# XinkeAE/Active-ORB-SLAM2

Hardware: AMD Instinct MI355X
Metric: frames/sec (extract+match+localBA) TUM 640x480 (higher is better)
Workload: dtype u8 (extract, match) + f64 (PoseOptimization, LocalBA)

## Files before the change

active-orb-slam2_amd/csrc/lba.hip:

```cpp
#include <dlfcn.h>

#include <chrono>
#include <cstdio>
#include <cstdlib>
#include <memory>
#include <numeric>
#include <atomic>
#include <condition_variable>
#include <functional>
#include <mutex>
#include <thread>

#include "lba_math.h"
#include "ldlt_reg.h"
#include "wave_ops.h"

namespace aos2 {

struct Cam {
    double fx, fy, cx, cy, bf;
    float bf_f;
    double delta_mono, delta_stereo;
};

// ... 64 lines not shown
    LdltForm ldlt_form;
    int hs_ld;
    LmState *st;
    const int32_t *abort_word;
    float *out_Tcw, *out_xyz;
    double *out_chi2;
    uint8_t *out_outlier;
};

static_assert(sizeof(LbaWin) == 520 && offsetof(LbaWin, st) == 472, "LbaWin's layout is fixed");

struct SchurTask {
    int32_t w;
    int32_t code;
};

typedef float flt4_t __attribute__((ext_vector_type(4)));
typedef int int4_t __attribute__((ext_vector_type(4)));
__device__ __forceinline__ void erec_load(const LbaWin &W, int a, flt4_t &lo, int4_t &hi)
{
    const EdgeRec *r = W.erec + a;
    lo = *reinterpret_cast<const flt4_t *>(r);
    hi = *(reinterpret_cast<const int4_t *>(r) + 1);
}
__device__ __forceinline__ void erec_store(const LbaWin &W, int a, flt4_t lo, int4_t hi)
{
    EdgeRec *r = W.erec + a;
    *reinterpret_cast<flt4_t *>(r) = lo;
    *(reinterpret_cast<int4_t *>(r) + 1) = hi;
}

__device__ inline bool lm_poll(LmState *st, const int32_t *abort_word, int seen = -1)
{
    st->polls++;
    if (st->stop_poll > 0) return true;
    const int a = seen >= 0 ? seen : abort_word ? __hip_atomic_load(abort_word, __ATOMIC_RELAXED, __HIP_MEMORY_SCOPE_SYSTEM) : 0;
    if (a || (st->stop_at_poll > 0 && st->polls >= st->stop_at_poll)) {
        st->stop_poll = st->polls;
        return true;
    }
    return false;
}

__device__ inline void lm_first_done(LmState *st, const int32_t *abort_word, int seen = -1)
{
    st->phase = 1;
    st->xmark = 0;
    if (lm_poll(st, abort_word, seen)) {
        st->phase = 3;
        return;
    }
    st->xmark = 1;
    st->n_active = 0;
}

template <int N>
__device__ __forceinline__ void workgroup_sum2(double v0, double v1, double *out0, double *out1)
{
    __shared__ double sh[2][N];
    sh[0][threadIdx.x] = v0;
    sh[1][threadIdx.x] = v1;
    __syncthreads();
#pragma unroll
    for (int s = N / 2; s > 0; s >>= 1) {
        if ((int)threadIdx.x < s) {
            sh[0][threadIdx.x] = sh[0][threadIdx.x] + sh[0][threadIdx.x + s];
            sh[1][threadIdx.x] = sh[1][threadIdx.x] + sh[1][threadIdx.x + s];
        }
        __syncthreads();
    }
    if (threadIdx.x == 0) {
        out0[blockIdx.x] = sh[0][0];
        out1[blockIdx.x] = sh[1][0];
    }
}

__global__ __launch_bounds__(256) void k_prepare(const LbaWin *__restrict__ wins, int stop_at_poll)
{
    const LbaWin &W = wins[blockIdx.y];
    const int i = blockIdx.x * 256 + threadIdx.x;
    if (i < W.n_poses) pose_from_Tcw(W.in_Tcw + 16 * (size_t)i, W.pose + 7 * (size_t)i);
    if (i < W.n_points)
        for (int d = 0; d < 3; ++d) W.point[3 * (size_t)i + d] = (double)W.in_xyz[3 * (size_t)i + d];
    if (i < W.n_edges) {
        for (int d = 0; d < 3; ++d) W.err[3 * (size_t)i + d] = 0.0;
        W.e_robust[i] = 1;
        W.e_level1[i] = 0;
        const int k = W.pt_k[i];
        const flt4_t lo = {W.in_obs[3 * (size_t)k], W.in_obs[3 * (size_t)k + 1], W.in_obs[3 * (size_t)k + 2], W.in_w[k]};
        const int4_t hi = {W.e_pose[k], W.pl_pos[k], (int)((W.e_stereo[k] ? kEdgeStereo : 0) | kEdgeRobust), 0};
        erec_store(W, i, lo, hi);
    }
    if (blockIdx.x == 0 && W.hs_ld == W.npad) {
        const int n = 6 * W.np, npad = W.npad;
        for (int q = threadIdx.x; q < (npad - n) * npad; q += 256) {
            const int r = n + q / npad, c = q % npad;
            W.Hs[(size_t)r * npad + c] = r == c ? 1.0 : 0.0;
        }
        for (int q = threadIdx.x; q < n * (npad - n); q += 256) {
            const int r = q / (npad - n), c = n + q % (npad - n);
            W.Hs[(size_t)r * npad + c] = 0.0;
        }
    }
    if (blockIdx.x == 0) {
        LmState *st = W.st;
        static_assert(sizeof(LmState) % 8 == 0, "LmState is cleared as 64-bit words");
        for (int k = threadIdx.x; k < (int)(sizeof(LmState) / 8); k += 256) reinterpret_cast<long long *>(st)[k] = 0;
        __syncthreads();
        if (threadIdx.x == 0) {
            st->iters_max[0] = W.iters1;
            st->iters_max[1] = W.iters2;
            st->polls = 1;
            st->stop_at_poll = stop_at_poll;
            st->n_active = W.n_edges;
            st->phase = 0;
            st->it = 0;
            if (st->iters_max[0] <= 0 || lm_poll(st, W.abort_word)) {
                st->iters_done[0] = 0;
                lm_first_done(st, W.abort_word);
            } else
                st->initp = 1;
        }
    }
}

__device__ __forceinline__ void edge_error(const Cam &cam, const double p[3], const double *obs, int stereo, double er[3])
{
    if (!stereo) {
        const double u = p[0] / p[2], v = p[1] / p[2];
        er[0] = obs[0] - (u * cam.fx + cam.cx);
        er[1] = obs[1] - (v * cam.fy + cam.cy);
        er[2] = 0;
    } else {
        const float invz = (float)(1.0 / p[2]);
        const double r0 = p[0] * invz * cam.fx + cam.cx;
        const double r1 = p[1] * invz * cam.fy + cam.cy;
        const double r2 = r0 - (double)__fmul_rn(cam.bf_f, invz);
        er[0] = obs[0] - r0;
        er[1] = obs[1] - r1;
        er[2] = obs[2] - r2;
    }
}

__device__ __forceinline__ double load_dev(const double *p)
{
    return __longlong_as_double((long long)__hip_atomic_load(reinterpret_cast<const unsigned long long *>(p), __ATOMIC_RELAXED,
                                                             __HIP_MEMORY_SCOPE_AGENT));
}
__device__ __forceinline__ void store_dev(double *p, double v)
{
    __hip_atomic_store(reinterpret_cast<unsigned long long *>(p), (unsigned long long)__double_as_longlong(v), __ATOMIC_RELAXED,
                       __HIP_MEMORY_SCOPE_AGENT);
}
__device__ __forceinline__ void canonical_sums(const LbaWin &W, bool with_scale, double &chi_out, double &scale_out)
{
    __shared__ double s_red[2][128];
    const int tid = threadIdx.x;
    if (tid < 128) {
        double c = 0, s2 = 0;
        for (int i0 = tid; i0 < W.nl; i0 += 128 * 16) {
            double v[16], w[16];
#pragma unroll
            for (int u = 0; u < 16; ++u) {
                const int i = i0 + 128 * u;
                v[u] = i < W.nl ? load_dev(W.part + i) : 0.0;
                w[u] = with_scale && i < W.nl ? load_dev(W.part + W.nl + i) : 0.0;
            }
#pragma unroll
            for (int u = 0; u < 16; ++u) {
                c += v[u];
                s2 += w[u];
            }
        }
        if (with_scale)
            for (int i = tid; i < 6 * W.np; i += 128) s2 += W.tmp[i];
        s_red[0][tid] = c;
        s_red[1][tid] = s2;
    }
    __syncthreads();
    for (int h = 64; h > 0; h >>= 1) {
        if (tid < h) {
            s_red[0][tid] += s_red[0][tid + h];
            s_red[1][tid] += s_red[1][tid + h];
        }
        __syncthreads();
    }
    chi_out = s_red[0][0];
    scale_out = s_red[1][0];
}
template <int NT>
__device__ __forceinline__ void lm_decide(const LbaWin &W)
{
    __shared__ int s_restore;
    LmState *st = W.st;
    const int flag_seen = threadIdx.x == 0 && W.abort_word ? __hip_atomic_load(W.abort_word, __ATOMIC_RELAXED, __HIP_MEMORY_SCOPE_SYSTEM) : 0;
    double tempChi, scale;
    canonical_sums(W, true, tempChi, scale);
    if (threadIdx.x == 0) {
        const int pass = st->phase == 0 ? 0 : 1;
        const bool ok2 = W.np == 0 || W.scal[3] != 0.0;
        if (!ok2) {
            tempChi = 1.7976931348623157e308;
            st->solver_failed++;
        }
        double rho = st->currentChi - tempChi;
        scale += 1e-3;
        rho /= scale;
        if (!ok2) rho = -1.0;
        const bool accepted = rho > 0 && isfinite(tempChi);
        if (st->ntr < 48) {
            st->tr_rho[st->ntr] = rho; st->tr_temp[st->ntr] = tempChi; st->tr_cur[st->ntr] = st->currentChi;
            st->tr_lambda[st->ntr] = st->lambda;
            st->ntr++;
        }
        if (accepted) {
            const double t3 = 2 * rho - 1;
            double alpha = 1. - t3 * t3 * t3;
            alpha = alpha < 2. / 3. ? alpha : 2. / 3.;
            const double scaleFactor = 1. / 3. > alpha ? 1. / 3. : alpha;
            st->lambda *= scaleFactor;
            st->ni = 2;
            st->currentChi = tempChi;
            st->err_at = 1;
        } else {
            st->lambda *= st->ni;
            st->ni *= 2;
            st->err_at = 2;
        }
        s_restore = accepted ? 0 : 1;
        st->qmax++;
        st->trials[pass]++;
        int lin = 0;
        const bool again = rho < 0 && st->qmax < 10 && !lm_poll(st, W.abort_word, flag_seen);
        if (!again) {
            bool term = st->qmax == 10 || rho == 0;
            if (!term) {
                if ((st->iniChi - st->currentChi) * 1e3 < st->iniChi)
                    st->nBad++;
                else
                    st->nBad = 0;
                term = st->nBad >= 3;
            }
            st->it++;
            bool more = st->it < st->iters_max[pass];
            if (more) more = !lm_poll(st, W.abort_word, flag_seen);
            if (more) more = !term;
            if (more) {
                st->qmax = 0;
                st->iniChi = st->currentChi;
                lin = accepted ? 1 : 0;
            } else {
                st->run = 0;
                st->iters_done[pass] = st->it;
                st->final_chi2 = st->currentChi;
                st->final_lambda = st->lambda;
                if (pass == 0)
                    lm_first_done(st, W.abort_word, flag_seen);
                else
                    st->phase = 3;
            }
        }
        st->lin = lin;
    }
    __syncthreads();
    if (s_restore)
        for (int i = threadIdx.x; i < W.est_n; i += NT) {
            const double trial = load_dev(W.pose + i);
            W.pose[i] = load_dev(W.bk + i);
            W.bk[i] = trial;
        }
}

template <int NT>
__device__ __forceinline__ void points_tail(const LbaWin &W)
{
    __shared__ int s_last;
    asm volatile("s_waitcnt vmcnt(0)" ::: "memory");
    __builtin_amdgcn_fence(__ATOMIC_RELEASE, "workgroup");
    __syncthreads();
    if (threadIdx.x == 0)
        s_last = __hip_atomic_fetch_add(&W.st->blocks_done, 1, __ATOMIC_RELAXED, __HIP_MEMORY_SCOPE_AGENT) == W.n_part - 1;
    __syncthreads();
    if (!s_last) return;
    __builtin_amdgcn_fence(__ATOMIC_ACQUIRE, "workgroup");
    if (threadIdx.x == 0) W.st->blocks_done = 0;
    lm_decide<NT>(W);
}

__device__ __forceinline__ void jac_pose(const Cam &cam, const double p[3], int stereo, double Jb[18])
{
    const double fx = cam.fx, fy = cam.fy, bf = cam.bf;
    const double iz = 1.0 / p[2], a = p[0] * iz, b = p[1] * iz, ab = a * b;
    Jb[0] = ab * fx;
    Jb[1] = -(1 + a * a) * fx;
    Jb[2] = b * fx;
    Jb[3] = -(iz * fx);
    Jb[4] = 0;
    Jb[5] = a * iz * fx;
    Jb[6] = (1 + b * b) * fy;
    Jb[7] = -(ab * fy);
    Jb[8] = -(a * fy);
    Jb[9] = 0;
    Jb[10] = -(iz * fy);
    Jb[11] = b * iz * fy;
#pragma unroll
    for (int i = 12; i < 18; ++i) Jb[i] = 0;
    if (stereo) {
        const double bfz2 = bf * (iz * iz);
        Jb[12] = Jb[0] - bfz2 * p[1];
        Jb[13] = Jb[1] + bfz2 * p[0];
        Jb[14] = Jb[2];
        Jb[15] = Jb[3];
        Jb[16] = 0;
        Jb[17] = Jb[5] - bfz2;
    }
}

__device__ __forceinline__ void jac_point(const Cam &cam, const double R[9], const double p[3], int stereo, double Ja[9])
{
    const double iz = 1.0 / p[2], a = p[0] * iz, b = p[1] * iz;
    const double fxz = cam.fx * iz, fyz = cam.fy * iz, afxz = a * fxz, bfyz = b * fyz;
#pragma unroll
    for (int c = 0; c < 3; ++c) {
        Ja[c] = afxz * R[6 + c] - fxz * R[c];
        Ja[3 + c] = bfyz * R[6 + c] - fyz * R[3 + c];
        Ja[6 + c] = 0;
    }
    if (stereo) {
        const double bfz2 = cam.bf * (iz * iz);
#pragma unroll
        for (int c = 0; c < 3; ++c) Ja[6 + c] = Ja[c] - bfz2 * R[6 + c];
    }
}

typedef double dbl4_t __attribute__((ext_vector_type(4)));
__device__ __forceinline__ void lrec_store(const LbaWin &W, int pos, const double p[3], double wo, int stereo, const double omr[3])
// ... 266 lines not shown
{
    const SchurTask tk = tasks[blockIdx.x];
    const LbaWin &W = wins[tk.w];
    if (!(solve ? W.st->run : W.st->initp)) return;
    const int l = tk.code * blockDim.x + threadIdx.x;
    const bool has = l < W.nl;
    int hp = 0, a0 = 0, a1 = 0, e0 = 0, e1 = 0;
    if (has) {
        hp = W.hpoint[l];
        e0 = W.pt_off[l];
        e1 = W.pt_off[l + 1];
        if (solve) {
            a0 = W.pl_off[l];
            a1 = W.pl_off[l + 1];
        }
    }
    const bool lds = walk_lds_bytes(W.n_poses, W.np) <= kWalkLdsBytes;
    if (lds) {
        walk_stage(W, walk_sm, solve != 0);
        if (has) points_walk_body<true>(W, l, solve, hp, a0, a1, e0, e1);
    } else if (has)
        points_walk_body<false>(W, l, solve, hp, a0, a1, e0, e1);
    if (solve) points_tail<128>(W);
}

__device__ __forceinline__ void edge_weights_of(const Cam &cam, const double er[3], double w, int robust, int stereo, double omr[3], double &wo)
{
    omr[0] = -(w * er[0]);
    omr[1] = -(w * er[1]);
    omr[2] = stereo ? -(w * er[2]) : 0.0;
    wo = w;
    if (robust) {
        double rho[2];
        robustify(edge_chi2(er, w, stereo ? 3 : 2), stereo ? cam.delta_stereo : cam.delta_mono, rho);
        wo = rho[1] * w;
        omr[0] *= rho[1];
        omr[1] *= rho[1];
        if (stereo) omr[2] *= rho[1];
    }
}
__device__ __forceinline__ void edge_weights(const LbaWin &W, int k, const double p[3], int stereo, double omr[3], double &wo)
{
    const double ob[3] = {(double)W.in_obs[3 * (size_t)k], (double)W.in_obs[3 * (size_t)k + 1], (double)W.in_obs[3 * (size_t)k + 2]};
    double er[3];
    edge_error(W.cam, p, ob, stereo, er);
    edge_weights_of(W.cam, er, (double)W.in_w[k], W.e_robust[k], stereo, omr, wo);
}

__device__ __forceinline__ void lin_points_body(const LbaWin &W, int blk)
{
    __shared__ double s_c[kLmBlock][kLmSlots][12 + 1];
    const int tid = threadIdx.x, ll = tid / kLmSlots, j = tid % kLmSlots;
    const int l = blk * kLmBlock + ll;
    const bool has = l < W.nl, leader = j == 0;
    double Xv[3] = {0, 0, 0};
    if (has) {
        const double *X = W.point + 3 * (size_t)W.hpoint[l];
        for (int r = 0; r < 3; ++r) Xv[r] = X[r];
    }
    double H[9] = {0, 0, 0, 0, 0, 0, 0, 0, 0}, bl[3] = {0, 0, 0};
    const int a0 = has ? W.pt_off[l] : 0, a1 = has ? W.pt_off[l + 1] : 0;
    for (int rd = 0; __syncthreads_or(a0 + kLmSlots * rd < a1); ++rd) {
        const int a = a0 + kLmSlots * rd + j;
        double cH[9] = {0, 0, 0, 0, 0, 0, 0, 0, 0}, cb[3] = {0, 0, 0};
        const int k = a < a1 ? W.pt_k[a] : -1;
        if (k >= 0 && !W.e_level1[k]) {
            const double *T = W.pose + 7 * (size_t)W.e_pose[k];
            const int stereo = W.e_stereo[k];
            double p[3], R[9];
            se3_map(T, Xv, p);
            rot_from_quat(T, R);
            double Ja[9];
            jac_point(W.cam, R, p, stereo, Ja);
            double omr[3], wo;
            edge_weights(W, k, p, stereo, omr, wo);
#pragma unroll
            for (int r = 0; r < 3; ++r) {
                cb[r] = Ja[r] * omr[0] + Ja[3 + r] * omr[1] + Ja[6 + r] * omr[2];
#pragma unroll
                for (int c = 0; c < 3; ++c) cH[r * 3 + c] = Ja[r] * wo * Ja[c] + Ja[3 + r] * wo * Ja[3 + c] + Ja[6 + r] * wo * Ja[6 + c];
            }
            const int pp = W.pl_pos[k];
            if (pp >= 0) lrec_store(W, pp, p, wo, stereo, omr);
        }
#pragma unroll
        for (int i = 0; i < 9; ++i) s_c[ll][j][i] = cH[i];
#pragma unroll
        for (int i = 0; i < 3; ++i) s_c[ll][j][9 + i] = cb[i];
        __syncthreads();
        if (leader) {
            const int m = min(kLmSlots, a1 - (a0 + kLmSlots * rd));
            for (int jj = 0; jj < m; ++jj) {
#pragma unroll
                for (int i = 0; i < 9; ++i) H[i] += s_c[ll][jj][i];
#pragma unroll
                for (int i = 0; i < 3; ++i) bl[i] += s_c[ll][jj][9 + i];
            }
        }
    }
    if (has && leader) {
        for (int i = 0; i < 9; ++i) W.Hll[9 * (size_t)l + i] = H[i];
        for (int i = 0; i < 3; ++i) W.b[6 * (size_t)W.np + 3 * (size_t)l + i] = bl[i];
    }
}

template <bool kLds>
__device__ __forceinline__ void lin_points_walk(const LbaWin &W, int l)
{
    const double *s_pose = walk_sm;
    const int e0 = W.pt_off[l], e1 = W.pt_off[l + 1];
    const double *X = W.point + 3 * (size_t)W.hpoint[l];
    const double Xv[3] = {X[0], X[1], X[2]};
    double H[9] = {0, 0, 0, 0, 0, 0, 0, 0, 0}, bl[3] = {0, 0, 0};
    for (int a = e0; a < e1; a += kWalkChunkLin) {
        flt4_t lo[kWalkChunkLin];
        int4_t hi[kWalkChunkLin];
        double T[kWalkChunkLin][7];
#pragma unroll
        for (int u = 0; u < kWalkChunkLin; ++u) erec_load(W, min(a + u, e1 - 1), lo[u], hi[u]);
#pragma unroll
        for (int u = 0; u < kWalkChunkLin; ++u)
#pragma unroll
            for (int i = 0; i < 7; ++i) T[u][i] = kLds ? s_pose[7 * hi[u].x + i] : W.pose[7 * (size_t)hi[u].x + i];
#pragma unroll
        for (int u = 0; u < kWalkChunkLin; ++u) {
            if (a + u >= e1) break;
            const uint32_t fl = (uint32_t)hi[u].z;
            if (fl & kEdgeLevel1) continue;
            const int stereo = fl & kEdgeStereo;
            const double ob[3] = {(double)lo[u].x, (double)lo[u].y, (double)lo[u].z};
            double p[3], R[9];
            se3_map(T[u], Xv, p);
            rot_from_quat(T[u], R);
            double Ja[9];
            jac_point(W.cam, R, p, stereo, Ja);
            double omr[3], wo;
            double res[3];
            edge_error(W.cam, p, ob, stereo, res);
            edge_weights_of(W.cam, res, (double)lo[u].w, (fl & kEdgeRobust) != 0, stereo, omr, wo);
#pragma unroll
            for (int r = 0; r < 3; ++r) {
                bl[r] += Ja[r] * omr[0] + Ja[3 + r] * omr[1] + Ja[6 + r] * omr[2];
#pragma unroll
                for (int c = 0; c < 3; ++c) H[r * 3 + c] += Ja[r] * wo * Ja[c] + Ja[3 + r] * wo * Ja[3 + c] + Ja[6 + r] * wo * Ja[6 + c];
            }
            if (hi[u].y >= 0) lrec_store(W, hi[u].y, p, wo, stereo, omr);
        }
    }
    asm volatile("" : "+v"(l));
    for (int i = 0; i < 9; ++i) W.Hll[9 * (size_t)l + i] = H[i];
    for (int i = 0; i < 3; ++i) W.b[6 * (size_t)W.np + 3 * (size_t)l + i] = bl[i];
}

template <int K, int NT = 256>
__device__ __forceinline__ double workgroup_sum_k256(double (&acc)[K], double *red , int n_items)
{
    const int row = threadIdx.x >> 4, wave = threadIdx.x >> 6;
    const int rows_used = min(NT / 16, (n_items + 15) >> 4);
    if (wave * 64 < n_items) {
        row_sums_scatter_f64<K>(acc);
        row_scatter_store<K>(acc, red + row * (K + 1));
    }
    __syncthreads();
    double sum = 0;
    if ((int)threadIdx.x < K)
        for (int r = 0; r < rows_used; ++r) sum += red[r * (K + 1) + threadIdx.x];
    return sum;
}

__device__ __forceinline__ void lin_poses_body(const LbaWin &W, int ph, int init)
{
    __shared__ double red[16 * 43];
    if (ph >= W.np) return;
    double T[7];
    {
        const double *Tp = W.pose + 7 * (size_t)W.hpose[ph];
#pragma unroll
        for (int i = 0; i < 7; ++i) T[i] = Tp[i];
    }
    if (threadIdx.x == 0) {
        double R[9];
        rot_from_quat(T, R);
#pragma unroll
        for (int i = 0; i < 9; ++i) W.Rl[9 * (size_t)ph + i] = R[i];
    }
    if (!init) return;
    double acc[42];
#pragma unroll
    for (int i = 0; i < 42; ++i) acc[i] = 0;
    for (int a = W.ps_off[ph] + threadIdx.x; a < W.ps_off[ph + 1]; a += 256) {
        const int k = W.ps_k[a];
        if (W.e_level1[k]) continue;
        const int stereo = W.e_stereo[k];
        double p[3], Jb[18], omr[3], wo;
        se3_map(T, W.point + 3 * (size_t)W.e_point[k], p);
        jac_pose(W.cam, p, stereo, Jb);
        edge_weights(W, k, p, stereo, omr, wo);
#pragma unroll
        for (int r = 0; r < 6; ++r) {
            acc[36 + r] += Jb[r] * omr[0] + Jb[6 + r] * omr[1] + Jb[12 + r] * omr[2];
#pragma unroll
            for (int c = 0; c < 6; ++c) acc[r * 6 + c] += Jb[r] * wo * Jb[c] + Jb[6 + r] * wo * Jb[6 + c] + Jb[12 + r] * wo * Jb[12 + c];
        }
    }
    const double sum = workgroup_sum_k256<42>(acc, red, W.ps_off[ph + 1] - W.ps_off[ph]);
    if (threadIdx.x < 36)
        W.Hpp[36 * (size_t)ph + threadIdx.x] = sum;
    else if (threadIdx.x < 42)
        W.b[6 * (size_t)ph + (threadIdx.x - 36)] = sum;
}

template <bool kWalk>
__global__ __launch_bounds__(256) __attribute__((amdgpu_waves_per_eu(3, 3))) void k_lin(const LbaWin *__restrict__ wins, const SchurTask *__restrict__ tasks, int init)
{
    const SchurTask tk = tasks[blockIdx.x];
    const LbaWin &W = wins[tk.w];
    if (!(init ? W.st->initp : W.st->lin)) return;
    const int blk = tk.code & 0x0fffffff;
    const bool keyframe = (tk.code >> 28) != 0;
    if (keyframe)
        lin_poses_body(W, blk, init);
    else if (kWalk) {
        const int l = blk * 256 + threadIdx.x;
        const bool has = l < W.nl;
        if (walk_lds_bytes(W.n_poses, W.np) <= kWalkLdsBytes) {
            walk_stage(W, walk_sm, false);
            if (has) lin_points_walk<true>(W, l);
        } else if (has)
            lin_points_walk<false>(W, l);
    } else
        lin_points_body(W, blk);
}

__global__ __launch_bounds__(1024) void k_lm_init(const LbaWin *__restrict__ wins)
{
    __shared__ double sh[1024];
    const LbaWin &W = wins[blockIdx.x];
    LmState *st = W.st;
    if (!st->initp) return;
    const int n6 = 6 * W.np, n = n6 + 3 * W.nl;
    double acc = 0;
    for (int i = threadIdx.x; i < n; i += 1024) {
        double v;
        if (i < n6)
            v = W.Hpp[36 * (size_t)(i / 6) + (i % 6) * 7];
        else {
            const int j = i - n6;
            v = W.Hll[9 * (size_t)(j / 3) + (j % 3) * 4];
        }
        acc = fmax(acc, fabs(v));
    }
    sh[threadIdx.x] = acc;
    __syncthreads();
    for (int s = 512; s > 0; s >>= 1) {
        if ((int)threadIdx.x < s) sh[threadIdx.x] = fmax(sh[threadIdx.x], sh[threadIdx.x + s]);
        __syncthreads();
    }
    for (int i = threadIdx.x; i < W.est_n; i += 1024) W.bk[i] = W.pose[i];
    double chi, unused;
    canonical_sums(W, false, chi, unused);
    if (threadIdx.x == 0) {
        st->currentChi = st->iniChi = chi;
        st->lambda = 1e-5 * sh[0];
        st->ni = 2;
        st->nBad = 0;
        st->it = 0;
        st->qmax = 0;
        st->initp = 0;
        st->lin = 0;
        st->run = 1;
        st->err_at = 1;
    }
}

constexpr int kSchurThreads = 256;
constexpr int kSchurDiag = 0, kSchurBig = 1, kSchurPack = 2;
__device__ __forceinline__ double sf(double a, double b, double c) { return a * b + c; }
template <bool kDiag>
__device__ __forceinline__ void schur_item(const LbaWin &W, int j, double lambda, int n6, const double *__restrict__ Ra_g,
                                           const double *__restrict__ Rb_g, double (&acc)[42])
{
    const int ka = W.it_ka[j], kb = W.it_kb[j], l = W.it_l[j];
    const dbl4_t rb = lrec_load(W, kb);
    const dbl4_t ra = kDiag ? rb : lrec_load(W, ka);
    double D[9], Dinv[9];
#pragma unroll
    for (int i = 0; i < 9; ++i) D[i] = W.Hll[9 * (size_t)l + i];
    D[0] += lambda; D[4] += lambda; D[8] += lambda;
    mat3_inverse(D, Dinv);
    double Ra[9], G[9];
#pragma unroll
    for (int i = 0; i < 9; ++i) Ra[i] = Ra_g[i];
    {
        double G0[9];
#pragma unroll
        for (int r = 0; r < 3; ++r)
#pragma unroll
            for (int c = 0; c < 3; ++c) G0[r * 3 + c] = sf(Ra[r * 3 + 2], Dinv[6 + c], sf(Ra[r * 3 + 1], Dinv[3 + c], Ra[r * 3] * Dinv[c]));
        if (kDiag) {
            const double *bl = W.b + n6 + 3 * (size_t)l;
            const double b0 = bl[0], b1 = bl[1], b2 = bl[2];
            const EdgeLin La = lrec_form(W.cam, ra);
            const double t[3] = {G0[0] * b0 + G0[1] * b1 + G0[2] * b2, G0[3] * b0 + G0[4] * b1 + G0[5] * b2, G0[6] * b0 + G0[7] * b1 + G0[8] * b2};
            double h[3];
            lrec_C(La, t, h);
            acc[36] += La.b * h[2] - h[1];
            acc[37] += h[0] - La.a * h[2];
            acc[38] += La.a * h[1] - La.b * h[0];
            acc[39] += La.iz * h[0];
            acc[40] += La.iz * h[1];
            acc[41] += La.iz * h[2];
        }
        double Rb[9];
#pragma unroll
        for (int i = 0; i < 9; ++i) Rb[i] = kDiag ? Ra[i] : Rb_g[i];
#pragma unroll
        for (int r = 0; r < 3; ++r)
#pragma unroll
            for (int c = 0; c < 3; ++c) G[r * 3 + c] = sf(G0[r * 3 + 2], Rb[c * 3 + 2], sf(G0[r * 3 + 1], Rb[c * 3 + 1], G0[r * 3] * Rb[c * 3]));
    }
    const EdgeLin La = lrec_form(W.cam, ra), Lb = kDiag ? La : lrec_form(W.cam, rb);
    double Q[9];
    {
        double CG[9];
#pragma unroll
        for (int c = 0; c < 3; ++c) {
            CG[c] = sf(La.C02, G[6 + c], La.C00 * G[c]);
            CG[3 + c] = sf(La.C12, G[6 + c], La.C11 * G[3 + c]);
            CG[6 + c] = sf(La.C22, G[6 + c], sf(La.C12, G[3 + c], La.C02 * G[c]));
        }
#pragma unroll
        for (int r = 0; r < 3; ++r) {
            Q[r * 3] = sf(CG[r * 3 + 2], Lb.C02, CG[r * 3] * Lb.C00);
            Q[r * 3 + 1] = sf(CG[r * 3 + 2], Lb.C12, CG[r * 3 + 1] * Lb.C11);
            Q[r * 3 + 2] = sf(CG[r * 3 + 2], Lb.C22, sf(CG[r * 3 + 1], Lb.C12, CG[r * 3] * Lb.C02));
        }
    }
    if (kDiag) {
        const double w = fabs(ra.w), fx2 = W.cam.fx * W.cam.fx, fy2 = W.cam.fy * W.cam.fy;
        const bool st = ra.w < 0.0;
        const double fs = st ? W.cam.fx : 0.0, c = st ? W.cam.bf * La.iz - La.a * W.cam.fx : 0.0;
        const double P00 = (fx2 + fs * fs) * w, P02 = (fs * c - La.a * fx2) * w, P11 = fy2 * w, P12 = -(La.b * fy2) * w;
        const double P22 = (La.a * La.a * fx2 + La.b * La.b * fy2 + c * c) * w;
        Q[0] -= P00; Q[2] -= P02; Q[4] -= P11; Q[5] -= P12; Q[6] -= P02; Q[7] -= P12; Q[8] -= P22;
    }
#pragma unroll
    for (int c = 0; c < 6; ++c) {
        double u[3];
#pragma unroll
        for (int r = 0; r < 3; ++r) {
            const double q0 = Q[r * 3], q1 = Q[r * 3 + 1], q2 = Q[r * 3 + 2];
            u[r] = c == 0 ? q1 - Lb.b * q2 : c == 1 ? Lb.a * q2 - q0 : c == 2 ? Lb.b * q0 - Lb.a * q1 : -(Lb.iz * Q[r * 3 + (c - 3)]);
        }
        acc[c] += u[1] - La.b * u[2];
        if (!kDiag || c >= 1) acc[6 + c] += La.a * u[2] - u[0];
        if (!kDiag || c >= 2) acc[12 + c] += La.b * u[0] - La.a * u[1];
        if (!kDiag || c >= 3) acc[18 + c] += -(La.iz * u[0]);
        if (!kDiag || c >= 4) acc[24 + c] += -(La.iz * u[1]);
        if (!kDiag || c >= 5) acc[30 + c] += -(La.iz * u[2]);
    }
    if (kDiag) {
        const double o[3] = {W.lomr[3 * (size_t)kb], W.lomr[3 * (size_t)kb + 1], W.lomr[3 * (size_t)kb + 2]};
        double bp[6] = {0, 0, 0, 0, 0, 0};
        lrec_bp(W.cam, ra, o, bp);
        acc[6] += bp[0]; acc[12] += bp[1]; acc[13] += bp[2]; acc[18] += bp[3]; acc[19] += bp[4]; acc[20] += bp[5];
    }
}

__device__ __forceinline__ void schur_store(const LbaWin &W, int i1, int i2, int e, double sum, double lambda)
{
    const bool diag = i1 == i2;
    if (e < 36) {
        double v = -sum;
        const int r = e / 6, c = e - 6 * r;
        if (diag && r == c) v += lambda;
        W.Hs[(size_t)(6 * i1 + r) * W.hs_ld + 6 * i2 + c] = v;
        if (!diag) W.Hs[(size_t)(6 * i2 + c) * W.hs_ld + 6 * i1 + r] = v;
    }
}

__global__ __launch_bounds__(kSchurThreads) __attribute__((amdgpu_waves_per_eu(3, 3)))
void k_schur(const LbaWin *__restrict__ wins, const SchurTask *__restrict__ tasks)
{
    constexpr int NT = kSchurThreads;
// ... 945 lines not shown
    W.erec = (EdgeRec *)(base + l.erec); W.npad = l.npad; W.ldlt_form = l.ldlt_form;
    W.hs_ld = l.npad;
    W.st = (LmState *)(base + l.st);
    W.abort_word = abort_word;
    W.out_Tcw = (float *)(base + l.out_Tcw); W.out_xyz = (float *)(base + l.out_xyz);
    W.out_outlier = base + l.out_outlier;
    W.out_chi2 = want_chi2 ? (double *)(base + l.out_chi2) : nullptr;
}


struct GroupDims {
    bool any_glob = false, any_reg = false;
    int mx_E = 0, mx_pts = 0, mx_npad_glob = 0, mx_npad_reg = 0;
    int walk_lds = 0;
    void add(const aos2_lba_problem_t &p, const Pass &S, const WinLayout &l)
    {
        if (S.np > 0) {
            if (l.ldlt_form == kLdltReg) {
                any_reg = true;
                mx_npad_reg = std::max(mx_npad_reg, l.npad);
            } else {
                any_glob = true;
                mx_npad_glob = std::max(mx_npad_glob, l.npad);
            }
        }
        mx_E = std::max(mx_E, p.n_edges);
        mx_pts = std::max(mx_pts, std::max(p.n_points, p.n_poses));
        if (walk_lds_bytes(p.n_poses, S.np) <= kWalkLdsBytes) walk_lds = std::max(walk_lds, walk_lds_bytes(p.n_poses, S.np));
    }
};

struct TaskLists {
    std::vector<SchurTask> schur, pts, lin;
    size_t size() const { return schur.size() + pts.size() + lin.size(); }
};

static void build_tasks(const std::vector<Pass> &passes, const std::vector<int> &ids, bool by_position, const LmLayout &lay, TaskLists &T, bool one_queue = false)
{
    auto wmap = [&](int k) { return by_position ? k : ids[k]; };
    std::vector<SchurTask> &tasks = T.schur;
    const int nwg = (int)ids.size();
    std::vector<int> order(nwg);
    std::iota(order.begin(), order.end(), 0);
    auto weight = [&](int k) { return passes[ids[k]].units.size(); };
    std::stable_sort(order.begin(), order.end(), [&](int a, int b) { return weight(a) > weight(b); });
    const int NX = nwg >= 8 && !one_queue ? 8 : 1;
    std::vector<std::vector<int>> xw(NX);
    std::vector<size_t> load(NX, 0);
    for (int k : order) {
        const int x = (int)(std::min_element(load.begin(), load.end()) - load.begin());
        xw[x].push_back(k);
        load[x] += weight(k);
    }
    std::vector<std::vector<SchurTask>> qx(NX);
    for (int x = 0; x < NX; ++x)
        for (size_t k = 0; k < xw[x].size(); k += 2) {
            const int a = xw[x][k], b = k + 1 < xw[x].size() ? xw[x][k + 1] : -1;
            const std::vector<int32_t> &ua = passes[ids[a]].units;
            static const std::vector<int32_t> none;
            const std::vector<int32_t> &ub = b >= 0 ? passes[ids[b]].units : none;
            for (size_t u = 0; u < std::max(ua.size(), ub.size()); ++u) {
                if (u < ua.size()) qx[x].push_back(SchurTask{wmap(a), ua[u]});
                if (u < ub.size()) qx[x].push_back(SchurTask{wmap(b), ub[u]});
            }
        }
    size_t mxq = 0;
    for (auto &q_ : qx) mxq = std::max(mxq, q_.size());
    tasks.assign(mxq * NX, SchurTask{-1, 0});
    for (int x = 0; x < NX; ++x)
        for (size_t k = 0; k < qx[x].size(); ++k) tasks[k * NX + x] = qx[x][k];
    int mx_pb = 0, mx_lb = 0, mx_k = 0;
    std::vector<int> npb(nwg), nlb(nwg);
    for (int k = 0; k < nwg; ++k) {
        const Pass &S = passes[ids[k]];
        npb[k] = lay.points_blocks(S);
        nlb[k] = lay.lin_blocks(S);
        mx_pb = std::max(mx_pb, npb[k]); mx_lb = std::max(mx_lb, nlb[k]); mx_k = std::max(mx_k, S.np);
    }
    T.pts.clear();
    T.lin.clear();
    for (int b = 0; b < mx_pb; ++b)
        for (int k = 0; k < nwg; ++k)
            if (b < npb[k]) T.pts.push_back(SchurTask{wmap(k), b});
    for (int b = 0; b < mx_lb; ++b)
        for (int k = 0; k < nwg; ++k)
            if (b < nlb[k]) T.lin.push_back(SchurTask{wmap(k), b});
    for (int kf = 0; kf < mx_k; ++kf)
        for (int k = 0; k < nwg; ++k)
            if (kf < passes[ids[k]].np) T.lin.push_back(SchurTask{wmap(k), (1 << 28) | kf});
}

struct DevTasks {
    const SchurTask *schur, *pts, *lin;
};
static DevTasks put_tasks(const TaskLists &T, uint8_t *host, const uint8_t *dev, size_t &o)
{
    DevTasks d;
    const std::vector<SchurTask> *lists[3] = {&T.schur, &T.pts, &T.lin};
    const SchurTask **where[3] = {&d.schur, &d.pts, &d.lin};
    for (int k = 0; k < 3; ++k) {
        *where[k] = (const SchurTask *)(dev + o);
        if (!lists[k]->empty()) memcpy(host + o, lists[k]->data(), sizeof(SchurTask) * lists[k]->size());
        o += sizeof(SchurTask) * lists[k]->size();
    }
    return d;
}

struct StreamSet {
    hipStream_t q, q2;
    hipEvent_t fork, join;
};
static StreamSet group_streams(const aos2_lba *s, int g)
{
    return g == 0 ? StreamSet{s->stream, s->stream2, s->ev_fork, s->ev_join} : StreamSet{s->stream_b, s->stream2_b, s->ev_fork_b, s->ev_join_b};
}

struct Prog : StreamSet {
    const LbaWin *wins, *blk;
    int nw;
    const SchurTask *schur, *pts, *lin;
    size_t n_schur, n_pts, n_lin;
    GroupDims D;
};
static Prog make_prog(const LbaWin *wins, const LbaWin *blk, int nw, const TaskLists &T, const DevTasks &d, const GroupDims &D, const StreamSet &Q)
{
    return Prog{Q, wins, blk, nw, d.schur, d.pts, d.lin, T.schur.size(), T.pts.size(), T.lin.size(), D};
}

struct LaunchCtx {
    aos2_lba *s;
    bool walk;
    bool stagger_pending;
};

static unsigned blocks(size_t n, int t) { return (unsigned)((n + t - 1) / t); }

static void enqueue_points(const LaunchCtx &C, const Prog &P, int solve)
{
    if (C.walk)
        hipLaunchKernelGGL(k_points_walk, dim3((unsigned)P.n_pts), dim3(128), (size_t)P.D.walk_lds, P.q, P.wins, P.pts, solve);
    else
        hipLaunchKernelGGL(k_points, dim3((unsigned)P.n_pts), dim3(256), 0, P.q, P.wins, P.pts, solve);
}
static void enqueue_lin(const LaunchCtx &C, const Prog &P, int init)
{
    if (!P.n_lin) return;
    if (C.walk)
        hipLaunchKernelGGL(k_lin<true>, dim3((unsigned)P.n_lin), dim3(256), (size_t)P.D.walk_lds, P.q, P.wins, P.lin, init);
    else
        hipLaunchKernelGGL(k_lin<false>, dim3((unsigned)P.n_lin), dim3(256), 0, P.q, P.wins, P.lin, init);
}
static void enqueue_init(const LaunchCtx &C, const Prog &P)
{
    enqueue_points(C, P, 0);
    enqueue_lin(C, P, 1);
    hipLaunchKernelGGL(k_lm_init, dim3(P.nw), dim3(1024), 0, P.q, P.blk);
}
static void enqueue_schur(const Prog &P)
{
    if (P.n_schur) hipLaunchKernelGGL(k_schur, dim3((unsigned)P.n_schur), dim3(kSchurThreads), 0, P.q, P.wins, P.schur);
}
static void enqueue_trial(LaunchCtx &C, const Prog &P, bool first_group)
{
    const GroupDims &D = P.D;
    enqueue_schur(P);
    if (first_group && C.stagger_pending) {
        (void)hipEventRecord(C.s->ev_stag, C.s->stream);
        (void)hipStreamWaitEvent(C.s->stream_b, C.s->ev_stag, 0);
        C.stagger_pending = false;
    }
    const bool both = D.any_glob && D.any_reg;
    if (both) {
        (void)hipEventRecord(P.fork, P.q);
        (void)hipStreamWaitEvent(P.q2, P.fork, 0);
    }
    enqueue_ldlt(P.blk, P.nw, D.any_reg ? D.mx_npad_reg : 0, D.any_glob ? D.mx_npad_glob : 0, both ? P.q2 : P.q, P.q);
    if (both) {
        (void)hipEventRecord(P.join, P.q2);
        (void)hipStreamWaitEvent(P.q, P.join, 0);
    }
    enqueue_points(C, P, 1);
    enqueue_lin(C, P, 0);
}
static void enqueue_transition(const Prog &P)
{
    hipLaunchKernelGGL(k_transition, dim3(blocks(P.D.mx_E, 256), P.nw), dim3(256), 0, P.q, P.blk);
}


static int settle_entry(const aos2_lba *s, const aos2_lba_problem_t *problems, aos2_lba_result_t *results, int n_problems, std::vector<int> &act, bool &want_chi2)
{
    want_chi2 = false;
    for (int w = 0; w < n_problems; ++w) {
        const aos2_lba_problem_t *p = problems + w;
        aos2_lba_result_t *r = results + w;
        if (p->n_poses <= 0 || p->n_points <= 0 || p->n_edges <= 0 || !p->pose_Tcw || !p->pose_fixed || !p->pose_id ||
            !p->point_xyz || !p->point_id || !p->edge_pose || !p->edge_point || !p->edge_obs || !p->edge_stereo ||
            !p->edge_inv_sigma2 || !r->pose_Tcw || !r->point_xyz) {
            set_error("bad LocalBA problem %d", w);
            return AOS2_ERR_ARG;
        }
        want_chi2 |= r->edge_chi2 != nullptr;
    }
    for (int w = 0; w < n_problems; ++w) {
        const aos2_lba_problem_t *p = problems + w;
        aos2_lba_result_t *r = results + w;
        r->iters_done_first = r->iters_done_second = 0;
        r->trials_first = r->trials_second = 0;
        r->final_chi2 = r->final_lambda = 0;
        r->ms_device = 0;
        r->polls = 1;
        r->stop_poll = 0;
        r->status = AOS2_OK;
        if (stop_requested(p) || s->debug_stop_at_poll == 1) {
            memcpy(r->pose_Tcw, p->pose_Tcw, sizeof(float) * 16 * p->n_poses);
            memcpy(r->point_xyz, p->point_xyz, sizeof(float) * 3 * p->n_points);
            if (r->edge_outlier) memset(r->edge_outlier, 0, p->n_edges);
            r->status = AOS2_ERR_STOPPED;
            r->stop_poll = 1;
        } else
            act.push_back(w);
    }
    return AOS2_OK;
}

static int deal_groups(const aos2_lba *s, const aos2_lba_problem_t *problems, std::vector<int> &act, int (&goff)[3])
{
    const int nw = (int)act.size();
    int G = s->window_groups ? s->window_groups : nw >= 16 ? 2 : 1;
    if (G > nw) G = 1;
    goff[0] = 0;
    goff[1] = goff[2] = nw;
    if (G == 2) {
        std::vector<int> order(act);
        std::stable_sort(order.begin(), order.end(), [&](int a, int b) { return problems[a].n_edges > problems[b].n_edges; });
        std::vector<int> g0, g1;
        for (size_t k = 0; k < order.size(); ++k) (((k & 3) == 0 || (k & 3) == 3) ? g0 : g1).push_back(order[k]);
        act = g0;
        act.insert(act.end(), g1.begin(), g1.end());
        goff[1] = (int)g0.size();
    }
    return G;
}

struct ArenaPlan {
    std::vector<WinLayout> L;
    size_t o_tasks, o_wins, staged_bytes, o_cont, cont_bytes, o_res, res_bytes, bytes;
};
static void plan_arena(const aos2_lba_problem_t *problems, const std::vector<int> &act, const std::vector<Pass> &passes, const LmLayout &lay, size_t n_all_tasks,
                       bool want_chi2, ArenaPlan &A)
{
    const int nw = (int)act.size();
    A.L.resize(nw);
    Bump B;
    for (int i = 0; i < nw; ++i) layout_staged(problems[act[i]], passes[i], B, A.L[i]);
    A.o_tasks = B.take(sizeof(SchurTask) * n_all_tasks + 8);
    A.o_wins = B.take(sizeof(LbaWin) * (size_t)nw);
    A.staged_bytes = B.size;
    size_t cont_tasks = 0, cont_max_units = 0;
    for (int i = 0; i < nw; ++i) {
        const Pass &S = passes[i];
        cont_max_units = std::max(cont_max_units, S.units.size());
        cont_tasks += S.units.size() + (size_t)lay.points_blocks(S) + (size_t)lay.lin_blocks(S) + (size_t)S.np;
    }
    cont_tasks += 8 * cont_max_units;
    A.cont_bytes = sizeof(LbaWin) * (size_t)nw + sizeof(SchurTask) * std::max(cont_tasks, n_all_tasks) + 64;
    A.o_cont = B.take(A.cont_bytes);
    for (int i = 0; i < nw; ++i) layout_scratch(problems[act[i]], passes[i], lay, B, A.L[i]);
    A.o_res = B.take(0);
    for (int i = 0; i < nw; ++i) layout_results(problems[act[i]], want_chi2, B, A.L[i]);
    A.res_bytes = B.size - A.o_res;
    A.bytes = B.size;
}

static int stage_and_upload(aos2_lba *s, WindowPool &pool, const aos2_lba_problem_t *problems, const std::vector<int> &act, const std::vector<Pass> &passes,
                            const ArenaPlan &A)
{
    const int nw = (int)act.size();
    uint8_t *base = s->arena.p, *hin = s->h_in.p;
    std::vector<uint8_t> up_fail(nw, 0);
    pool.run(nw, [&](int i) {
        stage_window(hin, A.L[i], problems[act[i]], passes[i]);
        const size_t r0 = A.L[i].in_Tcw, r1 = i + 1 < nw ? A.L[i + 1].in_Tcw : A.o_tasks;
        if (hipSetDevice(s->device) != hipSuccess || hipMemcpyAsync(base + r0, hin + r0, r1 - r0, hipMemcpyHostToDevice, s->stream) != hipSuccess)
            up_fail[i] = 1;
    });
    for (int i = 0; i < nw; ++i)
        if (up_fail[i]) {
            set_error("LocalBA: upload of window %d failed", act[i]);
            return AOS2_ERR_HIP;
        }
    return AOS2_OK;
}

static void enqueue_prepare(const LaunchCtx &C, const Prog &P)
{
    hipLaunchKernelGGL(k_prepare, dim3(blocks(std::max(P.D.mx_E, P.D.mx_pts), 256), P.nw), dim3(256), 0, P.q, P.blk, C.s->debug_stop_at_poll);
}

static void enqueue_program(LaunchCtx &C, const Prog &P, bool first_group, const int (&iters)[2], const int (&slots)[2])
{
    enqueue_prepare(C, P);
    for (int k = 0; k < 2; ++k) {
        if (k == 1) enqueue_transition(P);
        if (iters[k] > 0) {
            enqueue_init(C, P);
// ... 582 lines not shown
```

Before: 78380.

## Fuse LM initialization into linearization kernel with last-block reduction

On the walk path, the separate points-solve, linearize and LM-init launches are replaced by one kernel. It linearizes points and poses, computes per-point chi2 and diagonal maxima, and backs up poses. The last block to finish, detected with an atomic counter, reduces chi2 and the max diagonal and initializes the LM state. This removes two kernel launches and a 1024-thread pass over the Hessian diagonals. In exchange it adds an atomic completion-counter protocol and changes lambda initialization to use a max reduction.

```diff
diff --git a/active-orb-slam2_amd/csrc/lba.hip b/active-orb-slam2_amd/csrc/lba.hip
--- a/active-orb-slam2_amd/csrc/lba.hip
+++ b/active-orb-slam2_amd/csrc/lba.hip
@@ -240,6 +240,7 @@
     __hip_atomic_store(reinterpret_cast<unsigned long long *>(p), (unsigned long long)__double_as_longlong(v), __ATOMIC_RELAXED,
                        __HIP_MEMORY_SCOPE_AGENT);
 }
+template <bool kMax = false>
 __device__ __forceinline__ void canonical_sums(const LbaWin &W, bool with_scale, double &chi_out, double &scale_out)
 {
     __shared__ double s_red[2][128];
@@ -257,11 +258,11 @@
 #pragma unroll
             for (int u = 0; u < 16; ++u) {
                 c += v[u];
-                s2 += w[u];
+                s2 = kMax ? fmax(s2, w[u]) : s2 + w[u];
             }
         }
         if (with_scale)
-            for (int i = tid; i < 6 * W.np; i += 128) s2 += W.tmp[i];
+            for (int i = tid; i < 6 * W.np; i += 128) s2 = kMax ? fmax(s2, load_dev(W.tmp + i)) : s2 + W.tmp[i];
         s_red[0][tid] = c;
         s_red[1][tid] = s2;
     }
@@ -269,7 +270,7 @@
     for (int h = 64; h > 0; h >>= 1) {
         if (tid < h) {
             s_red[0][tid] += s_red[0][tid + h];
-            s_red[1][tid] += s_red[1][tid + h];
+            s_red[1][tid] = kMax ? fmax(s_red[1][tid], s_red[1][tid + h]) : s_red[1][tid] + s_red[1][tid + h];
         }
         __syncthreads();
     }
@@ -842,6 +843,67 @@
     for (int i = 0; i < 3; ++i) W.b[6 * (size_t)W.np + 3 * (size_t)l + i] = bl[i];
 }
 
+template <bool kLds>
+__device__ __forceinline__ void lin_points_walk_setup(const LbaWin &W, int l)
+{
+    const double *s_pose = walk_sm;
+    const int e0 = W.pt_off[l], e1 = W.pt_off[l + 1];
+    const double *X = W.point + 3 * (size_t)W.hpoint[l];
+    const double Xv[3] = {X[0], X[1], X[2]};
+    double H[9] = {0, 0, 0, 0, 0, 0, 0, 0, 0}, bl[3] = {0, 0, 0}, chi = 0;
+    for (int a = e0; a < e1; a += kWalkChunkLin) {
+        flt4_t lo[kWalkChunkLin];
+        int4_t hi[kWalkChunkLin];
+        double T[kWalkChunkLin][7];
+#pragma unroll
+        for (int u = 0; u < kWalkChunkLin; ++u) erec_load(W, min(a + u, e1 - 1), lo[u], hi[u]);
+#pragma unroll
+        for (int u = 0; u < kWalkChunkLin; ++u)
+#pragma unroll
+            for (int i = 0; i < 7; ++i) T[u][i] = kLds ? s_pose[7 * hi[u].x + i] : W.pose[7 * (size_t)hi[u].x + i];
+#pragma unroll
+        for (int u = 0; u < kWalkChunkLin; ++u) {
+            if (a + u >= e1) break;
+            const uint32_t fl = (uint32_t)hi[u].z;
+            if (fl & kEdgeLevel1) continue;
+            const int stereo = fl & kEdgeStereo;
+            const double ob[3] = {(double)lo[u].x, (double)lo[u].y, (double)lo[u].z};
+            double p[3], R[9];
+            se3_map(T[u], Xv, p);
+            rot_from_quat(T[u], R);
+            double Ja[9];
+            jac_point(W.cam, R, p, stereo, Ja);
+            double res[3];
+            edge_error(W.cam, p, ob, stereo, res);
+            const double w = (double)lo[u].w;
+            double omr[3] = {-(w * res[0]), -(w * res[1]), stereo ? -(w * res[2]) : 0.0}, wo = w;
+            double c = edge_chi2(res, w, stereo ? 3 : 2);
+            if (fl & kEdgeRobust) {
+                double rho[2];
+                robustify(c, stereo ? W.cam.delta_stereo : W.cam.delta_mono, rho);
+                c = rho[0];
+                wo = rho[1] * w;
+                omr[0] *= rho[1];
+                omr[1] *= rho[1];
+                if (stereo) omr[2] *= rho[1];
+            }
+            chi += c;
+#pragma unroll
+            for (int r = 0; r < 3; ++r) {
+                bl[r] += Ja[r] * omr[0] + Ja[3 + r] * omr[1] + Ja[6 + r] * omr[2];
+#pragma unroll
+                for (int c2 = 0; c2 < 3; ++c2) H[r * 3 + c2] += Ja[r] * wo * Ja[c2] + Ja[3 + r] * wo * Ja[3 + c2] + Ja[6 + r] * wo * Ja[6 + c2];
+            }
+            if (hi[u].y >= 0) lrec_store(W, hi[u].y, p, wo, stereo, omr);
+        }
+    }
+    asm volatile("" : "+v"(l));
+    for (int i = 0; i < 9; ++i) W.Hll[9 * (size_t)l + i] = H[i];
+    for (int i = 0; i < 3; ++i) W.b[6 * (size_t)W.np + 3 * (size_t)l + i] = bl[i];
+    store_dev(W.part + l, chi);
+    store_dev(W.part + W.nl + l, fmax(fmax(fmax(0.0, fabs(H[0])), fabs(H[4])), fabs(H[8])));
+}
+
 template <int K, int NT = 256>
 __device__ __forceinline__ double workgroup_sum_k256(double (&acc)[K], double *red , int n_items)
 {
@@ -858,10 +920,10 @@
     return sum;
 }
 
-__device__ __forceinline__ void lin_poses_body(const LbaWin &W, int ph, int init)
+__device__ __forceinline__ double lin_poses_body(const LbaWin &W, int ph, int init)
 {
     __shared__ double red[16 * 43];
-    if (ph >= W.np) return;
+    if (ph >= W.np) return 0.0;
     double T[7];
     {
         const double *Tp = W.pose + 7 * (size_t)W.hpose[ph];
@@ -874,7 +936,7 @@
 #pragma unroll
         for (int i = 0; i < 9; ++i) W.Rl[9 * (size_t)ph + i] = R[i];
     }
-    if (!init) return;
+    if (!init) return 0.0;
     double acc[42];
 #pragma unroll
     for (int i = 0; i < 42; ++i) acc[i] = 0;
@@ -898,6 +960,7 @@
         W.Hpp[36 * (size_t)ph + threadIdx.x] = sum;
     else if (threadIdx.x < 42)
         W.b[6 * (size_t)ph + (threadIdx.x - 36)] = sum;
+    return sum;
 }
 
 template <bool kWalk>
@@ -920,6 +983,52 @@
             lin_points_walk<false>(W, l);
     } else
         lin_points_body(W, blk);
+}
+
+__global__ __launch_bounds__(256) __attribute__((amdgpu_waves_per_eu(3, 3))) void k_lin_setup(const LbaWin *__restrict__ wins, const SchurTask *__restrict__ tasks)
+{
+    __shared__ int s_last;
+    const SchurTask tk = tasks[blockIdx.x];
+    const LbaWin &W = wins[tk.w];
+    LmState *st = W.st;
+    if (!st->initp) return;
+    const int blk = tk.code & 0x0fffffff;
+    const int lin_blocks = (W.nl + 255) / 256;
+    if ((tk.code >> 28) != 0) {
+        const double sum = lin_poses_body(W, blk, 1);
+        if (threadIdx.x < 36 && threadIdx.x % 7 == 0) store_dev(W.tmp + 6 * (size_t)blk + threadIdx.x / 7, fabs(sum));
+    } else {
+        const int l = blk * 256 + threadIdx.x;
+        for (int i = l; i < W.est_n; i += lin_blocks * 256) W.bk[i] = W.pose[i];
+        if (walk_lds_bytes(W.n_poses, W.np) <= kWalkLdsBytes) {
+            walk_stage(W, walk_sm, false);
+            if (l < W.nl) lin_points_walk_setup<true>(W, l);
+        } else if (l < W.nl)
+            lin_points_walk_setup<false>(W, l);
+    }
+    asm volatile("s_waitcnt vmcnt(0)" ::: "memory");
+    __builtin_amdgcn_fence(__ATOMIC_RELEASE, "workgroup");
+    __syncthreads();
+    if (threadIdx.x == 0)
+        s_last = __hip_atomic_fetch_add(&st->blocks_done, 1, __ATOMIC_RELAXED, __HIP_MEMORY_SCOPE_AGENT) == lin_blocks + W.np - 1;
+    __syncthreads();
+    if (!s_last) return;
+    __builtin_amdgcn_fence(__ATOMIC_ACQUIRE, "workgroup");
+    double chi, max_diag;
+    canonical_sums<true>(W, true, chi, max_diag);
+    if (threadIdx.x == 0) {
+        st->blocks_done = 0;
+        st->currentChi = st->iniChi = chi;
+        st->lambda = 1e-5 * max_diag;
+        st->ni = 2;
+        st->nBad = 0;
+        st->it = 0;
+        st->qmax = 0;
+        st->initp = 0;
+        st->lin = 0;
+        st->run = 1;
+        st->err_at = 1;
+    }
 }
 
 __global__ __launch_bounds__(1024) void k_lm_init(const LbaWin *__restrict__ wins)
@@ -2171,6 +2280,10 @@
 }
 static void enqueue_init(const LaunchCtx &C, const Prog &P)
 {
+    if (C.walk) {
+        hipLaunchKernelGGL(k_lin_setup, dim3((unsigned)P.n_lin), dim3(256), (size_t)P.D.walk_lds, P.q, P.wins, P.lin);
+        return;
+    }
     enqueue_points(C, P, 0);
     enqueue_lin(C, P, 1);
     hipLaunchKernelGGL(k_lm_init, dim3(P.nw), dim3(1024), 0, P.q, P.blk);
```

Result: slower. 77400 (-1.3%).
